# wkh923/m3pc

Measured on AMD Instinct MI355X. Metric: MPC plan-steps/sec (N=1024, H=16, hopper-medium-v2); independent plan steps, 3 in flight, higher is better.
Workload: dtype bf16; 1 GPU; hopper-medium-v2 shapes (S=11,A=3) rtg_guiding N=1024 H=16 T=32 bf16 candidate pass + fp32 policy pass + fp32 re-score (arg-max and multinomial draw certified under the calibrated bound delta, 8.4 candidates re-scored on average); 3 independent plan steps in flight (policy pass / candidate pass / re-score of neighbouring steps on different streams); window resident in HBM; candidates_per_gpu=1024, global_candidates=1024, horizon=16, traj_length=32, steps_in_flight=3, settle_steps=24, parallelism=1 GPU

## Files before the change

m3pc_amd/csrc/attn_bf16.hip:

```cpp
#include <cstdio>

#include "kernels.h"

namespace m3pc {

typedef float f32x16 __attribute__((ext_vector_type(16)));
typedef __bf16 bf16x8 __attribute__((ext_vector_type(8)));
typedef __bf16 bf16x4 __attribute__((ext_vector_type(4)));
typedef unsigned int u32x4 __attribute__((ext_vector_type(4)));
typedef short s16x4 __attribute__((ext_vector_type(4)));
typedef short s16x8 __attribute__((ext_vector_type(8)));
typedef float f32x4v __attribute__((ext_vector_type(4)));

template <int HDT, int NCH>
__global__ __launch_bounds__(256) void attn_bf16_kernel(AttnP p) {
    constexpr int HD = HDT * 32;
    constexpr int ROWB = HD * 2 + 16;
    constexpr int NS = HD / 16;
    constexpr int CPR = HD / 8;
    extern __shared__ __attribute__((aligned(16))) char lds[];

    const int tid = threadIdx.x, lane = tid & 63, wid = tid >> 6;
    const int nthr = blockDim.x, nw = nthr >> 6;
    const int b = blockIdx.x, head = blockIdx.y, qg = blockIdx.z;
// ... 190 lines not shown
    const int Lk = p.L1 + p.L2;
    const int l31 = lane & 31, lh = lane >> 5;
    const bf16_t* Qb = (const bf16_t*)p.Q + b * p.q_bstride + head * HD;
    const bf16_t* K1 = (const bf16_t*)p.K1 + b * p.kv1_bstride + head * HD;
    const bf16_t* V1 = (const bf16_t*)p.V1 + b * p.kv1_bstride + head * HD;
    const bf16_t* K2 = p.K2 ? (const bf16_t*)p.K2 + head * HD : nullptr;
    const bf16_t* V2 = p.V2 ? (const bf16_t*)p.V2 + head * HD : nullptr;
    const u32x4 zero4 = {0u, 0u, 0u, 0u};
    const int Lq1p = (p.Lq + 31) & ~31;
    const bf16_t* Q2b = p.Q2 ? (const bf16_t*)p.Q2 + head * HD : nullptr;

    const int qi = q0 + wid * 32 + l31;
    const bf16_t* qrow = nullptr;
    if (qi < p.Lq)
        qrow = Qb + (long long)qi * p.ldq;
    else if (Q2b && qi >= Lq1p && qi - Lq1p < p.Lq2)
        qrow = Q2b + (long long)(qi - Lq1p) * p.ldq2;
    u32x4 qf[NS];
#pragma unroll
    for (int s = 0; s < NS; ++s) {
        qf[s] = zero4;
        if (qrow) qf[s] = *(const u32x4*)(qrow + 16 * s + 8 * lh);
    }
    f32x16 sacc[NKT];
#pragma unroll
    for (int jt = 0; jt < NKT; ++jt)
#pragma unroll
        for (int e = 0; e < 16; ++e) sacc[jt][e] = 0.f;
#pragma unroll
    for (int pr = 0; pr < NKT / 2; ++pr) {
        u32x4 kf[2][NS];
#pragma unroll
        for (int t = 0; t < 2; ++t) {
            const int j = (2 * pr + t) * 32 + l31;
            const bf16_t* krow = j < p.L1 ? K1 + (long long)j * p.ldkv1 : (j < Lk ? K2 + (long long)(j - p.L1) * p.ldkv2 : nullptr);
#pragma unroll
            for (int s = 0; s < NS; ++s) {
                kf[t][s] = zero4;
                if (krow) kf[t][s] = *(const u32x4*)(krow + 16 * s + 8 * lh);
            }
        }
#pragma unroll
        for (int t = 0; t < 2; ++t)
            if ((2 * pr + t) * 32 < Lk) {
#pragma unroll
                for (int s = 0; s < NS; ++s)
                    sacc[2 * pr + t] = __builtin_amdgcn_mfma_f32_32x32x16_bf16(__builtin_bit_cast(bf16x8, kf[t][s]),
                                                                               __builtin_bit_cast(bf16x8, qf[s]), sacc[2 * pr + t], 0, 0, 0);
            }
    }
    u32x4 vv[VPT];
#pragma unroll
    for (int i = 0; i < VPT; ++i) {
        const int x = tid + i * NTHR, r = x / CPR, kc = x % CPR;
        vv[i] = zero4;
        if (r < p.L1)
            vv[i] = *(const u32x4*)(V1 + (long long)r * p.ldkv1 + kc * 8);
        else if (r < Lk)
            vv[i] = *(const u32x4*)(V2 + (long long)(r - p.L1) * p.ldkv2 + kc * 8);
    }

    float m = -INFINITY;
#pragma unroll
    for (int jt = 0; jt < NKT; ++jt)
#pragma unroll
        for (int e = 0; e < 16; ++e) {
            const int j = jt * 32 + (e & 3) + 8 * (e >> 2) + 4 * lh;
            const float v = (j < Lk) ? sacc[jt][e] * p.scale : -INFINITY;
            sacc[jt][e] = v;
            m = fmaxf(m, v);
        }
    m = fmaxf(m, __shfl_xor(m, 32));
    float l = 0.f;
#pragma unroll
    for (int jt = 0; jt < NKT; ++jt)
#pragma unroll
        for (int e = 0; e < 16; ++e) {
            const float v = __builtin_amdgcn_exp2f((sacc[jt][e] - m) * 1.44269504088896340736f);
            sacc[jt][e] = v;
            l += v;
        }
    l += __shfl_xor(l, 32);
    float inv = 1.0f / l;
    if (p.pre_m) {
        float mp = -INFINITY, lp = 0.f;
        if (qi < p.Lq) {
            mp = p.pre_m[head * p.Lq + qi];
            lp = p.pre_l[head * p.Lq + qi];
        }
        const float mt = fmaxf(m, mp);
        const float a = __builtin_amdgcn_exp2f((m - mt) * 1.44269504088896340736f);
        const float bs = __builtin_amdgcn_exp2f((mp - mt) * 1.44269504088896340736f);
        const float lt = l * a + lp * bs;
        inv = a / lt;
        if (lh == 0) fbuf[wid * 32 + l31] = bs / lt;
    }
#pragma unroll
    for (int i = 0; i < VPT; ++i) {
        const int x = tid + i * NTHR, r = x / CPR, kc = x % CPR;
        *(u32x4*)(lds + r * ROWB + kc * 16) = vv[i];
    }
    __syncthreads();

    f32x16 oacc[HDT];
#pragma unroll
    for (int d = 0; d < HDT; ++d)
#pragma unroll
        for (int e = 0; e < 16; ++e) oacc[d][e] = 0.f;
    const int gi = lane & 15;
    const int tr_off = (gi >> 2) * ROWB + (((lane >> 4) & 1) * 16 + (gi & 3) * 4) * 2;
#pragma unroll
    for (int jt = 0; jt < NKT; ++jt) {
        if (jt * 32 < Lk) {
#pragma unroll
            for (int s2 = 0; s2 < 2; ++s2) {
                bf16x8 pa;
#pragma unroll
                for (int e = 0; e < 8; ++e) pa[e] = (bf16_t)(sacc[jt][8 * s2 + e] * inv);
                const int kb = jt * 32 + 16 * s2 + 4 * lh;
#pragma unroll
                for (int d = 0; d < HDT; ++d) {
                    const char* base = lds + kb * ROWB + d * 64 + tr_off;
                    const s16x4 v0 = __builtin_amdgcn_ds_read_tr16_b64_v4i16((s16x4 __attribute__((address_space(3)))*)(base));
                    const s16x4 v1 =
                        __builtin_amdgcn_ds_read_tr16_b64_v4i16((s16x4 __attribute__((address_space(3)))*)(base + 8 * ROWB));
                    const s16x8 vb = __builtin_shufflevector(v0, v1, 0, 1, 2, 3, 4, 5, 6, 7);
                    oacc[d] = __builtin_amdgcn_mfma_f32_32x32x16_bf16(pa, __builtin_bit_cast(bf16x8, vb), oacc[d], 0, 0, 0);
                }
            }
        }
    }
    bf16_t* Ob = (bf16_t*)p.O + b * p.o_bstride + head * HD;
#pragma unroll
    for (int e = 0; e < 16; ++e) {
        const int i = q0 + wid * 32 + (e & 3) + 8 * (e >> 2) + 4 * lh;
        int orow = -1;
        if (i < p.Lq)
            orow = p.orow1 + i;
        else if (Q2b && i >= Lq1p && i - Lq1p < p.Lq2)
            orow = p.orow2 + i - Lq1p;
        if (orow >= 0) {
            if (p.pre_m) {
                const float f = fbuf[i - q0];
                const float* po = p.pre_O + ((long long)head * p.Lq + i) * HD;
#pragma unroll
                for (int d = 0; d < HDT; ++d) oacc[d][e] = fmaf(f, po[d * 32 + l31], oacc[d][e]);
            }
#pragma unroll
            for (int d = 0; d < HDT; ++d) Ob[(long long)orow * p.ldo + d * 32 + l31] = (bf16_t)oacc[d][e];
        }
    }
}
namespace {
constexpr int APIPE_NR = 52, APIPE_IMG = APIPE_NR * 256, APIPE_BUF = 3 * APIPE_IMG;
}
template <int N1, int SH>
__global__ __launch_bounds__(192, 2) void attn_bf16_pipe_kernel(AttnP p, int n_items) {
#if defined(__HIP_DEVICE_COMPILE__)
    constexpr int HD = 128, NS = 8, HDT = 4;
    constexpr int Lk = N1 + SH;
    constexpr int NP_OWN = (N1 + 3) / 4, NP_SH = SH ? (Lk + 3) / 4 - N1 / 4 : 0;
    constexpr int NDMA = NP_OWN + 2 * (NP_OWN + NP_SH);
    static_assert(NDMA <= 63 && Lk <= APIPE_NR && (SH == 0 || (SH == 32 && N1 <= APIPE_NR - 32)), "shapes");
    extern __shared__ __attribute__((aligned(16))) char lds[];
    typedef __attribute__((address_space(3))) void* lptr_t;
    const int tid = threadIdx.x, lane = tid & 63;
    const int wid = __builtin_amdgcn_readfirstlane(tid >> 6);
    const int l31 = lane & 31, lh = lane >> 5;
    constexpr int QROW0 = SH ? 32 : 0;

    {
        const u32x4 z = {0u, 0u, 0u, 0u};
        constexpr int NZ = (APIPE_NR - Lk) * 16;
        for (int i = tid; i < 2 * NZ; i += 192) *(u32x4*)(lds + (i / NZ) * APIPE_BUF + Lk * 256 + (i % NZ) * 16) = z;
    }
    const int r4 = lane >> 4, c16 = lane & 15;
    const int n_mine = ((int)blockIdx.x < n_items) ? (n_items - 1 - (int)blockIdx.x) / (int)gridDim.x + 1 : 0;
    const int stride = gridDim.x;
    asm volatile("s_waitcnt lgkmcnt(0)\n\ts_barrier" ::: "memory");

    if (wid == 2) {
        auto voff = [&](int ld, int odd) { return (unsigned)(r4 * ld * 2 + ((c16 ^ (4 * odd + r4)) << 4)); };
        const unsigned vq[2] = {voff(p.ldq, 0), voff(p.ldq, 1)};
        const unsigned vk[2] = {voff(p.ldkv1, 0), voff(p.ldkv1, 1)}, vk2[2] = {voff(p.ldkv2, 0), voff(p.ldkv2, 1)};
        auto seg_dma = [&](const bf16_t* src, int ld, const unsigned (&v)[2], char* img, auto r0_c, auto l_c, auto aux_c) {
            constexpr int R0 = decltype(r0_c)::value, L = decltype(l_c)::value, AUX = decltype(aux_c)::value;
            if (L == 0) return;
            const __amdgpu_buffer_rsrc_t rs = __builtin_amdgcn_make_buffer_rsrc((void*)(src - (long long)R0 * ld), 0, (unsigned)((R0 + L) * ld * 2), 0x00020000);
#pragma unroll
            for (int pc = R0 / 4; pc <= (R0 + L - 1) / 4; ++pc) {
                const bool lo = 4 * pc >= R0 ? true : 4 * pc + r4 >= R0;
                const bool hi = 4 * pc + 3 < R0 + L ? true : 4 * pc + r4 < R0 + L;
                if (lo && hi) __builtin_amdgcn_raw_ptr_buffer_load_lds(rs, (lptr_t)(img + pc * 1024), 16, v[pc & 1], pc * 4 * ld * 2, 0, AUX);
            }
        };
        using I0 = std::integral_constant<int, 0>;
        auto issue = [&](int it, int buf) {
            if (p.no_pipe == 3) return;
            const int b = it >> 2, head = it & 3;
            char* const B = lds + buf * APIPE_BUF;
            using AS = std::integral_constant<int, M3PC_STREAM_AUX>;
            seg_dma((const bf16_t*)p.K1 + b * p.kv1_bstride + head * HD, p.ldkv1, vk, B + APIPE_IMG, I0{}, std::integral_constant<int, N1>{}, AS{});
            seg_dma((const bf16_t*)p.K2 + head * HD, p.ldkv2, vk2, B + APIPE_IMG, std::integral_constant<int, N1>{}, std::integral_constant<int, SH>{}, I0{});
            seg_dma((const bf16_t*)p.Q + b * p.q_bstride + head * HD, p.ldq, vq, B + 2 * APIPE_IMG, std::integral_constant<int, QROW0>{}, std::integral_constant<int, N1>{}, AS{});
            seg_dma((const bf16_t*)p.V1 + b * p.kv1_bstride + head * HD, p.ldkv1, vk, B, I0{}, std::integral_constant<int, N1>{}, AS{});
            seg_dma((const bf16_t*)p.V2 + head * HD, p.ldkv2, vk2, B, std::integral_constant<int, N1>{}, std::integral_constant<int, SH>{}, I0{});
        };
        if (n_mine > 0) issue(blockIdx.x, 0);
        if (n_mine > 1) issue(blockIdx.x + stride, 1);
        for (int k = 0; k < n_mine; ++k) {
            if (k == 0 && n_mine > 1) asm volatile("s_waitcnt vmcnt(%0)" ::"n"(NDMA) : "memory");
            else asm volatile("s_waitcnt vmcnt(0)" ::: "memory");
            asm volatile("s_barrier" ::: "memory");
            if (k >= 1 && k + 1 < n_mine) issue(blockIdx.x + (k + 1) * stride, (k + 1) & 1);
            asm volatile("s_barrier" ::: "memory");
        }
        return;
    }
    const int qi = wid * 32 + l31;
    const int sw = l31 & 7;
    const int gi = lane & 15;
    long long st_[8] = {0, 0, 0, 0, 0, 0, 0, 0};
    u32x4 qf[NS];
    if (SH && wid == 1) {
        const bf16_t* qrow = (const bf16_t*)p.Q2 + (blockIdx.x % p.n_head) * HD + (long long)l31 * p.ldq2 + 8 * lh;
#pragma unroll
        for (int s = 0; s < NS; ++s) qf[s] = *(const u32x4*)(qrow + 16 * s);
    }
    for (int k = 0; k < n_mine; ++k) {
        const int it = blockIdx.x + k * stride;
        const char* const B = lds + (k & 1) * APIPE_BUF;
        asm volatile("s_barrier" ::: "memory");
        if (p.stamps && k == 2) st_[0] = __builtin_readcyclecounter();
        if (p.no_pipe == 2) {
            asm volatile("s_barrier" ::: "memory");
            continue;
        }
        const unsigned vbase = (unsigned)(uintptr_t)(const __attribute__((address_space(3))) char*)B;
        const char* const Ki = B + APIPE_IMG;
        const char* const Qi = B + 2 * APIPE_IMG;
        if (SH == 0 || wid == 0) {
#pragma unroll
            for (int s = 0; s < NS; ++s) qf[s] = *(const u32x4*)(Qi + (QROW0 + qi) * 256 + (((2 * s + lh) ^ sw) << 4));
        }
        f32x16 sacc[2];
#pragma unroll
        for (int t = 0; t < 2; ++t)
#pragma unroll
            for (int e = 0; e < 16; ++e) sacc[t][e] = 0.f;
#pragma unroll
        for (int s = 0; s < NS; ++s)
#pragma unroll
            for (int t = 0; t < 2; ++t) {
                const u32x4 kf = *(const u32x4*)(Ki + (32 * t + l31) * 256 + (((2 * s + lh) ^ sw) << 4));
                sacc[t] = __builtin_amdgcn_mfma_f32_32x32x16_bf16(__builtin_bit_cast(bf16x8, kf), __builtin_bit_cast(bf16x8, qf[s]), sacc[t], 0, 0, 0);
            }
        asm volatile("" : "+v"(sacc[0]), "+v"(sacc[1]));
        if (p.stamps && k == 2) st_[1] = __builtin_readcyclecounter();
        float m = -INFINITY;
#pragma unroll
        for (int jt = 0; jt < 2; ++jt)
#pragma unroll
            for (int e = 0; e < 16; ++e) {
                if (jt * 32 + (e & 3) + 8 * (e >> 2) >= Lk) continue;
                const int j = jt * 32 + (e & 3) + 8 * (e >> 2) + 4 * lh;
                const float v = (jt * 32 + (e & 3) + 8 * (e >> 2) + 4 < Lk || j < Lk) ? sacc[jt][e] * p.scale : -INFINITY;
                sacc[jt][e] = v;
                m = fmaxf(m, v);
            }
        m = fmaxf(m, __shfl_xor(m, 32));
        float l = 0.f;
#pragma unroll
        for (int jt = 0; jt < 2; ++jt)
#pragma unroll
            for (int e = 0; e < 16; ++e) {
                if (jt * 32 + (e & 3) + 8 * (e >> 2) >= Lk) {
                    sacc[jt][e] = 0.f;
                    continue;
                }
                const float v = __builtin_amdgcn_exp2f((sacc[jt][e] - m) * 1.44269504088896340736f);
                sacc[jt][e] = v;
                l += v;
            }
        l += __shfl_xor(l, 32);
        const float inv = 1.0f / l;
        asm volatile("" : "+v"(l));
        if (p.stamps && k == 2) st_[2] = __builtin_readcyclecounter();
        f32x16 oacc[HDT];
#pragma unroll
        for (int d = 0; d < HDT; ++d)
#pragma unroll
            for (int e = 0; e < 16; ++e) oacc[d][e] = 0.f;
        s16x4 tv[2][2 * HDT];
        auto tr_reads = [&](int n, s16x4 (&v)[2 * HDT]) {
            const int kr = 16 * n + 4 * lh + (gi >> 2);
#pragma unroll
            for (int d = 0; d < HDT; ++d) {
                const int bo = d * 64 + ((lane >> 4) & 1) * 32 + (gi & 3) * 8;
                const unsigned a0 = vbase + kr * 256 + ((((bo >> 4) ^ (kr & 7)) << 4) | (bo & 15));
                const unsigned a1 = vbase + (kr + 8) * 256 + ((((bo >> 4) ^ ((kr + 8) & 7)) << 4) | (bo & 15));
                asm volatile("ds_read_b64_tr_b16 %0, %1" : "=v"(v[2 * d]) : "v"(a0));
                asm volatile("ds_read_b64_tr_b16 %0, %1" : "=v"(v[2 * d + 1]) : "v"(a1));
            }
        };
        tr_reads(0, tv[0]);
#pragma unroll
        for (int n = 0; n < 4; ++n) {
            const int jt = n >> 1, s2 = n & 1;
            bf16x8 pa;
#pragma unroll
            for (int e = 0; e < 8; ++e) pa[e] = (bf16_t)(sacc[jt][8 * s2 + e] * inv);
            s16x4(&cur)[2 * HDT] = tv[n & 1];
            if (n < 3) {
                tr_reads(n + 1, tv[(n + 1) & 1]);
                asm volatile("s_waitcnt lgkmcnt(8)" : "+v"(cur[0]), "+v"(cur[1]), "+v"(cur[2]), "+v"(cur[3]), "+v"(cur[4]), "+v"(cur[5]), "+v"(cur[6]), "+v"(cur[7]));
            } else {
                asm volatile("s_waitcnt lgkmcnt(0)" : "+v"(cur[0]), "+v"(cur[1]), "+v"(cur[2]), "+v"(cur[3]), "+v"(cur[4]), "+v"(cur[5]), "+v"(cur[6]), "+v"(cur[7]));
            }
#pragma unroll
            for (int d = 0; d < HDT; ++d) {
                const s16x8 vb = __builtin_shufflevector(cur[2 * d], cur[2 * d + 1], 0, 1, 2, 3, 4, 5, 6, 7);
                oacc[d] = __builtin_amdgcn_mfma_f32_32x32x16_bf16(__builtin_bit_cast(bf16x8, vb), pa, oacc[d], 0, 0, 0);
            }
        }
        asm volatile("" : "+v"(oacc[0]), "+v"(oacc[1]), "+v"(oacc[2]), "+v"(oacc[3]));
        if (p.stamps && k == 2) st_[3] = __builtin_readcyclecounter();
        {
            char* const Oi = (char*)Qi;
            const int orow_i = SH == 0 ? qi : (wid == 0 ? 32 + qi : qi - 32);
            if (SH == 0 ? qi < APIPE_NR : (wid == 1 || qi < N1)) {
#pragma unroll
                for (int d = 0; d < HDT; ++d)
#pragma unroll
                    for (int q = 0; q < 4; ++q) {
                        bf16x4 w;
#pragma unroll
                        for (int i = 0; i < 4; ++i) w[i] = (bf16_t)oacc[d][4 * q + i];
                        *(bf16x4*)(Oi + orow_i * 256 + (((4 * d + q) ^ (orow_i & 7)) << 4) + 8 * lh) = w;
                    }
            }
        }
        if (p.stamps && k == 2) st_[4] = __builtin_readcyclecounter();
        constexpr int NPC_LO = 8, NPC_HI = APIPE_NR / 4 - 8;
        const bool low_rows = SH == 0 ? wid == 0 : wid == 1;
        u32x4 ov[NPC_LO];
#pragma unroll
        for (int j = 0; j < NPC_LO; ++j) {
            const int pc = low_rows ? j : (j < NPC_HI ? 8 + j : 8 + NPC_HI - 1);
            ov[j] = *(const u32x4*)(Qi + (4 * pc + r4) * 256 + c16 * 16);
        }
        asm volatile("s_waitcnt lgkmcnt(0)\n\ts_barrier" ::: "memory");
        if (p.stamps && k == 2) st_[5] = __builtin_readcyclecounter();
        {
            const int b = it >> 2, head = it & 3;
            const __amdgpu_buffer_rsrc_t o_rs = __builtin_amdgcn_make_buffer_rsrc(
                (void*)((bf16_t*)p.O + b * p.o_bstride + head * HD), 0, 0x7fffffffu, 0x00020000);
#pragma unroll
            for (int j = 0; j < NPC_LO; ++j) {
                const int pc = low_rows ? j : (j < NPC_HI ? 8 + j : 8 + NPC_HI - 1);
                const int row = 4 * pc + r4;
                const unsigned off = row < Lk ? (unsigned)((SH ? row : p.orow1 + row) * p.ldo * 2) : 0x80000000u;
                __builtin_amdgcn_raw_buffer_store_b128(ov[j], o_rs, off + ((c16 ^ (row & 7)) << 4), 0, M3PC_STREAM_AUX);
            }
        }
        if (p.stamps && k == 2) st_[6] = __builtin_readcyclecounter();
    }
    if (p.stamps && (int)blockIdx.x == 37 && lane == 0)
        for (int i = 0; i < 7; ++i) p.stamps[wid * 8 + i] = st_[i];
#endif
}
template <int N1>
__global__ __launch_bounds__(192, 1) void attn_bf16_pipe_dec_kernel(AttnP p, int n_items) {
#if defined(__HIP_DEVICE_COMPILE__)
    constexpr int HD = 128, NS = 8, HDT = 4;
    constexpr int Lk = N1;
    constexpr int NPC = (N1 + 3) / 4;
    constexpr int NDMA = 2 * 2 * NPC;
    constexpr int DBUF = 2 * APIPE_IMG;
    static_assert(NDMA <= 63 && Lk <= APIPE_NR, "shapes");
    extern __shared__ __attribute__((aligned(16))) char lds[];
    typedef __attribute__((address_space(3))) void* lptr_t;
    const int tid = threadIdx.x, lane = tid & 63;
    const int wid = __builtin_amdgcn_readfirstlane(tid >> 6);
    const int l31 = lane & 31, lh = lane >> 5;
    {
        const u32x4 z = {0u, 0u, 0u, 0u};
        constexpr int NZ = (APIPE_NR - Lk) * 16;
        for (int i = tid; i < 4 * NZ; i += 192) *(u32x4*)(lds + (i / NZ) * DBUF + Lk * 256 + (i % NZ) * 16) = z;
    }
    const int r4 = lane >> 4, c16 = lane & 15;
    const int stride = gridDim.x;
    const int n_mine = ((int)blockIdx.x < n_items) ? (n_items - 1 - (int)blockIdx.x) / stride + 1 : 0;
    const int n_rounds = (n_mine + 1) / 2;
    const int head = blockIdx.x & 3;
    asm volatile("s_waitcnt lgkmcnt(0)\n\ts_barrier" ::: "memory");

    if (wid == 2) {
        const unsigned v[2] = {(unsigned)(r4 * p.ldkv1 * 2 + ((c16 ^ r4) << 4)), (unsigned)(r4 * p.ldkv1 * 2 + ((c16 ^ (4 + r4)) << 4))};
        auto issue = [&](int r) {
            if (p.no_pipe == 3) return;
#pragma unroll
            for (int w = 0; w < 2; ++w) {
                int j = 2 * r + w;
                j = j < n_mine ? j : n_mine - 1;
                const int it = blockIdx.x + stride * j;
                char* const B = lds + (2 * w + (r & 1)) * DBUF;
                const bf16_t* kb = (const bf16_t*)p.K1 + (long long)(it >> 2) * p.kv1_bstride + head * HD;
                const bf16_t* vb = (const bf16_t*)p.V1 + (long long)(it >> 2) * p.kv1_bstride + head * HD;
                const __amdgpu_buffer_rsrc_t krs = __builtin_amdgcn_make_buffer_rsrc((void*)kb, 0, (unsigned)(N1 * p.ldkv1 * 2), 0x00020000);
                const __amdgpu_buffer_rsrc_t vrs = __builtin_amdgcn_make_buffer_rsrc((void*)vb, 0, (unsigned)(N1 * p.ldkv1 * 2), 0x00020000);
#pragma unroll
                for (int pc = 0; pc < NPC; ++pc) {
                    const bool ok = 4 * pc + 3 < N1 ? true : 4 * pc + r4 < N1;
                    if (ok) {
                        __builtin_amdgcn_raw_ptr_buffer_load_lds(krs, (lptr_t)(B + APIPE_IMG + pc * 1024), 16, v[pc & 1], pc * 4 * p.ldkv1 * 2, 0, M3PC_STREAM_AUX);
                        __builtin_amdgcn_raw_ptr_buffer_load_lds(vrs, (lptr_t)(B + pc * 1024), 16, v[pc & 1], pc * 4 * p.ldkv1 * 2, 0, M3PC_STREAM_AUX);
                    }
                }
            }
        };
        if (n_rounds > 0) issue(0);
        if (n_rounds > 1) issue(1);
        for (int r = 0; r < n_rounds; ++r) {
            if (r == 0 && n_rounds > 1) asm volatile("s_waitcnt vmcnt(%0)" ::"n"(NDMA) : "memory");
            else asm volatile("s_waitcnt vmcnt(0)" ::: "memory");
            asm volatile("s_barrier" ::: "memory");
            if (r >= 1 && r + 1 < n_rounds) issue(r + 1);
            asm volatile("s_barrier" ::: "memory");
        }
        return;
    }
    const int qi = l31;
    const int sw = l31 & 7;
    const int gi = lane & 15;
    u32x4 qf[NS];
    {
        const bf16_t* qrow = (const bf16_t*)p.Q + head * HD + (long long)(qi < p.Lq ? qi : 0) * p.ldq + 8 * lh;
#pragma unroll
        for (int s = 0; s < NS; ++s) qf[s] = *(const u32x4*)(qrow + 16 * s);
    }
    float mp = -INFINITY, lp = 0.f;
    f32x4v po[HDT][4];
    if (qi < p.Lq) {
        mp = p.pre_m[head * p.Lq + qi];
        lp = p.pre_l[head * p.Lq + qi];
    }
    {
        const float* prow = p.pre_O + ((long long)head * p.Lq + (qi < p.Lq ? qi : 0)) * HD + 4 * lh;
#pragma unroll
        for (int d = 0; d < HDT; ++d)
#pragma unroll
            for (int q = 0; q < 4; ++q) po[d][q] = *(const f32x4v*)(prow + d * 32 + 8 * q);
    }
    const unsigned ooff_base = qi < p.Lq ? 0u : 0x80000000u;
    (void)ooff_base;
    for (int r = 0; r < n_rounds; ++r) {
        const int j = 2 * r + wid;
        const bool have = j < n_mine;
        const int it = blockIdx.x + stride * (have ? j : 0);
        const char* const B = lds + (2 * wid + (r & 1)) * DBUF;
        asm volatile("s_barrier" ::: "memory");
        if (have && p.no_pipe != 2) {
            const unsigned vbase = (unsigned)(uintptr_t)(const __attribute__((address_space(3))) char*)B;
            const char* const Ki = B + APIPE_IMG;
            f32x16 sacc[2];
#pragma unroll
            for (int t = 0; t < 2; ++t)
#pragma unroll
                for (int e = 0; e < 16; ++e) sacc[t][e] = 0.f;
#pragma unroll
            for (int s = 0; s < NS; ++s)
#pragma unroll
                for (int t = 0; t < 2; ++t) {
                    const u32x4 kf = *(const u32x4*)(Ki + (32 * t + l31) * 256 + (((2 * s + lh) ^ sw) << 4));
                    sacc[t] = __builtin_amdgcn_mfma_f32_32x32x16_bf16(__builtin_bit_cast(bf16x8, kf), __builtin_bit_cast(bf16x8, qf[s]), sacc[t], 0, 0, 0);
                }
            float m = -INFINITY;
#pragma unroll
            for (int jt = 0; jt < 2; ++jt)
#pragma unroll
                for (int e = 0; e < 16; ++e) {
                    if (jt * 32 + (e & 3) + 8 * (e >> 2) >= Lk) continue;
                    const int jj = jt * 32 + (e & 3) + 8 * (e >> 2) + 4 * lh;
                    const float v = (jt * 32 + (e & 3) + 8 * (e >> 2) + 4 < Lk || jj < Lk) ? sacc[jt][e] * p.scale : -INFINITY;
                    sacc[jt][e] = v;
                    m = fmaxf(m, v);
                }
            m = fmaxf(m, __shfl_xor(m, 32));
            float l = 0.f;
#pragma unroll
            for (int jt = 0; jt < 2; ++jt)
#pragma unroll
                for (int e = 0; e < 16; ++e) {
                    if (jt * 32 + (e & 3) + 8 * (e >> 2) >= Lk) {
                        sacc[jt][e] = 0.f;
                        continue;
                    }
                    const float v = __builtin_amdgcn_exp2f((sacc[jt][e] - m) * 1.44269504088896340736f);
                    sacc[jt][e] = v;
                    l += v;
                }
            l += __shfl_xor(l, 32);
            const float mt = fmaxf(m, mp);
            const float a = __builtin_amdgcn_exp2f((m - mt) * 1.44269504088896340736f);
            const float bs = __builtin_amdgcn_exp2f((mp - mt) * 1.44269504088896340736f);
            const float lt = l * a + lp * bs;
            const float inv = a / lt;
            const float fpre = bs / lt;
            f32x16 oacc[HDT];
#pragma unroll
            for (int d = 0; d < HDT; ++d)
#pragma unroll
                for (int e = 0; e < 16; ++e) oacc[d][e] = 0.f;
            s16x4 tv[2][2 * HDT];
            auto tr_reads = [&](int n, s16x4 (&v)[2 * HDT]) {
                const int kr = 16 * n + 4 * lh + (gi >> 2);
#pragma unroll
                for (int d = 0; d < HDT; ++d) {
                    const int bo = d * 64 + ((lane >> 4) & 1) * 32 + (gi & 3) * 8;
                    const unsigned a0 = vbase + kr * 256 + ((((bo >> 4) ^ (kr & 7)) << 4) | (bo & 15));
                    const unsigned a1 = vbase + (kr + 8) * 256 + ((((bo >> 4) ^ ((kr + 8) & 7)) << 4) | (bo & 15));
// ... 411 lines not shown
            }
        float m = -INFINITY;
#pragma unroll
        for (int jt = 0; jt < NKT; ++jt)
#pragma unroll
            for (int e = 0; e < 16; ++e) {
                if (jt * 32 + (e & 3) + 8 * (e >> 2) >= Lk) continue;
                const int j = jt * 32 + (e & 3) + 8 * (e >> 2) + 4 * lh;
                const float v = (jt * 32 + (e & 3) + 8 * (e >> 2) + 4 < Lk || j < Lk) ? sacc[jt][e] * p.scale : -INFINITY;
                sacc[jt][e] = v;
                m = fmaxf(m, v);
            }
        m = fmaxf(m, __shfl_xor(m, 32));
        float l = 0.f;
#pragma unroll
        for (int jt = 0; jt < NKT; ++jt)
#pragma unroll
            for (int e = 0; e < 16; ++e) {
                if (jt * 32 + (e & 3) + 8 * (e >> 2) >= Lk) {
                    sacc[jt][e] = 0.f;
                    continue;
                }
                const float v = __builtin_amdgcn_exp2f((sacc[jt][e] - m) * 1.44269504088896340736f);
                sacc[jt][e] = v;
                l += v;
            }
        l += __shfl_xor(l, 32);
        float inv = 1.0f / l, fpre = 0.f;
        if constexpr (PRE) {
            const float mt = fmaxf(m, mp);
            const float a = __builtin_amdgcn_exp2f((m - mt) * 1.44269504088896340736f);
            const float bs = __builtin_amdgcn_exp2f((mp - mt) * 1.44269504088896340736f);
            const float lt = l * a + lp * bs;
            inv = a / lt;
            fpre = bs / lt;
        }
        u32x4 pa[NSTEP];
#pragma unroll
        for (int n = 0; n < NSTEP; ++n) {
            bf16x8 w;
#pragma unroll
            for (int e = 0; e < 8; ++e) w[e] = (bf16_t)(sacc[n >> 1][8 * (n & 1) + e] * inv);
            pa[n] = __builtin_bit_cast(u32x4, w);
            asm volatile("" : "+v"(pa[n]));
        }
        f32x16 oacc[HDT];
#pragma unroll
        for (int d = 0; d < HDT; ++d)
#pragma unroll
            for (int e = 0; e < 16; ++e) oacc[d][e] = 0.f;
        s16x4 tv[2][2 * HDT];
        unsigned tb[HDT];
        {
            const int kr = 4 * lh + (gi >> 2);
#pragma unroll
            for (int d = 0; d < HDT; ++d) {
                const int bo = d * 64 + ((lane >> 4) & 1) * 32 + (gi & 3) * 8;
                tb[d] = vbase + kr * 256 + ((((bo >> 4) ^ (kr & 7)) << 4) | (bo & 15));
            }
        }
        auto tr_reads = [](auto n_c, const unsigned (&tb)[HDT], s16x4 (&v)[2 * HDT]) {
            constexpr int n = decltype(n_c)::value;
#pragma unroll
            for (int d = 0; d < HDT; ++d) {
                asm volatile("ds_read_b64_tr_b16 %0, %1 offset:%2" : "=v"(v[2 * d]) : "v"(tb[d]), "n"(n * 4096));
                asm volatile("ds_read_b64_tr_b16 %0, %1 offset:%2" : "=v"(v[2 * d + 1]) : "v"(tb[d]), "n"(n * 4096 + 2048));
            }
        };
        tr_reads(std::integral_constant<int, 0>{}, tb, tv[0]);
        static_for<NSTEP>([&](auto n_c) {
            constexpr int n = decltype(n_c)::value;
            s16x4(&cur)[2 * HDT] = tv[n & 1];
            if constexpr (n < NSTEP - 1) {
                tr_reads(std::integral_constant<int, n + 1>{}, tb, tv[(n + 1) & 1]);
                asm volatile("s_waitcnt lgkmcnt(8)" : "+v"(cur[0]), "+v"(cur[1]), "+v"(cur[2]), "+v"(cur[3]), "+v"(cur[4]), "+v"(cur[5]), "+v"(cur[6]), "+v"(cur[7]));
            } else {
                asm volatile("s_waitcnt lgkmcnt(0)" : "+v"(cur[0]), "+v"(cur[1]), "+v"(cur[2]), "+v"(cur[3]), "+v"(cur[4]), "+v"(cur[5]), "+v"(cur[6]), "+v"(cur[7]));
            }
#pragma unroll
            for (int d = 0; d < HDT; ++d) {
                const s16x8 vb = __builtin_shufflevector(cur[2 * d], cur[2 * d + 1], 0, 1, 2, 3, 4, 5, 6, 7);
                oacc[d] = __builtin_amdgcn_mfma_f32_32x32x16_bf16(__builtin_bit_cast(bf16x8, vb), __builtin_bit_cast(bf16x8, pa[n]), oacc[d], 0, 0, 0);
            }
        });
        {
            char* const Oi = (char*)Qi;
            if (qrow_i < WPIPE_NR) {
#pragma unroll
                for (int d = 0; d < HDT; ++d)
#pragma unroll
                    for (int q = 0; q < 4; ++q) {
                        bf16x4 w;
#pragma unroll
                        for (int i = 0; i < 4; ++i) w[i] = (bf16_t)(PRE ? fmaf(fpre, po[PRE ? d : 0][q][i], oacc[d][4 * q + i]) : oacc[d][4 * q + i]);
                        *(bf16x4*)(Oi + qrow_i * 256 + (((4 * d + q) ^ sw) << 4) + 8 * lh) = w;
                    }
            }
        }
        u32x4 ov[8];
#pragma unroll
        for (int j = 0; j < 8; ++j) {
            const int pc = 8 * wid + j < WPIPE_NR / 4 ? 8 * wid + j : WPIPE_NR / 4 - 1;
            ov[j] = *(const u32x4*)(Qi + (4 * pc + r4) * 256 + c16 * 16);
        }
        asm volatile("s_waitcnt lgkmcnt(0)\n\ts_barrier" ::: "memory");
        {
            const __amdgpu_buffer_rsrc_t o_rs = __builtin_amdgcn_make_buffer_rsrc(
                (void*)((bf16_t*)p.O + (long long)(it >> 2) * p.o_bstride + head * HD), 0, 0x7fffffffu, 0x00020000);
#pragma unroll
            for (int j = 0; j < 8; ++j) {
                const int pc = 8 * wid + j;
                const int row = 4 * pc + r4;
                const unsigned off = pc < WPIPE_NR / 4 && row < n_out ? (unsigned)((SHQ && !PRE ? row : p.orow1 + row) * p.ldo * 2) : 0x80000000u;
                __builtin_amdgcn_raw_buffer_store_b128(ov[j], o_rs, off + ((c16 ^ (row & 7)) << 4), 0, 0);
            }
        }
    }
#endif
}
template <typename K>
static bool lds_opt_in(K kernel, int bytes) {
    static bool done[64] = {}, ok[64] = {};
    int dev = 0;
    if (hipGetDevice(&dev) != hipSuccess || dev < 0 || dev >= 64) return false;
    if (!done[dev]) {
        ok[dev] = hipFuncSetAttribute((const void*)kernel, hipFuncAttributeMaxDynamicSharedMemorySize, bytes) == hipSuccess;
        done[dev] = true;
    }
    return ok[dev];
}
template <int N1, int N2>
static bool launch_pipe_mix(const AttnP& p, hipStream_t st) {
    const int n_items = p.batch * p.n_head;
    const int grid = n_items < 256 ? n_items : 256;
    constexpr int LDSB = 2 * ((N2 + 3) / 4) * 1024 + 4 * (2 * APIPE_IMG + 1024);
    static_assert(LDSB <= 160 * 1024, "LDS");
    if (!lds_opt_in(attn_bf16_pipe_mix_kernel<N1, N2>, LDSB)) return false;
    M3PC_ATTN_PICK(23);
    hipLaunchKernelGGL((attn_bf16_pipe_mix_kernel<N1, N2>), dim3(grid), dim3(192), LDSB, st, p, n_items);
    return true;
}
template <int N1>
static bool launch_pipe_dec(const AttnP& p, hipStream_t st) {
    const int n_items = p.batch * p.n_head;
    const int grid = n_items < 256 ? n_items : 256;
    if (!lds_opt_in(attn_bf16_pipe_dec_kernel<N1>, 8 * APIPE_IMG)) return false;
    M3PC_ATTN_PICK(22);
    hipLaunchKernelGGL((attn_bf16_pipe_dec_kernel<N1>), dim3(grid), dim3(192), 8 * APIPE_IMG, st, p, n_items);
    return true;
}
template <int N1, int SH>
static bool launch_pipe(const AttnP& p, hipStream_t st) {
    const int n_items = p.batch * p.n_head;
    int cap = 512;
#ifdef M3PC_LAB
    static const int env_cap = M3PC_ENV("M3PC_ATTN_PIPE_GRID") ? atoi(M3PC_ENV("M3PC_ATTN_PIPE_GRID")) : 0;
    if (env_cap > 0) cap = env_cap;
#endif
    cap -= cap % p.n_head;
    const int grid = n_items < cap ? n_items : cap;
    if (!lds_opt_in(attn_bf16_pipe_kernel<N1, SH>, 2 * APIPE_BUF)) return false;
    size_t lds_bytes = 2 * APIPE_BUF;
#ifdef M3PC_LAB
    static const int env_lds = M3PC_ENV("M3PC_ATTN_PIPE_LDS") ? atoi(M3PC_ENV("M3PC_ATTN_PIPE_LDS")) : 0;
    if (env_lds > 0) lds_bytes = env_lds;
#endif
    M3PC_ATTN_PICK(SH == 0 ? 20 : 21);
    hipLaunchKernelGGL((attn_bf16_pipe_kernel<N1, SH>), dim3(grid), dim3(192), lds_bytes, st, p, n_items);
    return true;
}
static bool wide_off() {
    static const bool off = M3PC_ENV("M3PC_NO_ATTN_PIPE_WIDE") != nullptr;
    return off;
}
template <int NQ1, int SHQ, int NK1, int SHK, bool PRE>
static bool launch_pipe_wide(const AttnP& p, hipStream_t st) {
    const int n_items = p.batch * p.n_head;
    const int grid = n_items < 256 ? n_items : 256;
    if (!lds_opt_in(attn_bf16_pipe_wide_kernel<NQ1, SHQ, NK1, SHK, PRE>, WPIPE_LDS)) return false;
    constexpr int NTHR = ((NQ1 + SHQ + 31) / 32 + 1) * 64;
    M3PC_ATTN_PICK(PRE ? 26 : SHQ == 0 ? 24 : 25);
    hipLaunchKernelGGL((attn_bf16_pipe_wide_kernel<NQ1, SHQ, NK1, SHK, PRE>), dim3(grid), dim3(NTHR), WPIPE_LDS, st, p, n_items);
    return true;
}
static bool try_pipe(const AttnP& p, hipStream_t st) {
    if (p.hd != 128 || p.n_head != 4 || p.no_pipe == 1 || p.batch * p.n_head < 1024) return false;
    if (p.pre_m) {
        if (p.q_bstride != 0 || p.Q2 || p.K2 || p.Lq < 1 || p.L2 != 0 || !p.pre_l || !p.pre_O) return false;
        if (((uintptr_t)p.Q | (uintptr_t)p.K1 | (uintptr_t)p.V1 | (uintptr_t)p.O | (uintptr_t)p.pre_O) & 15) return false;
        if ((p.ldq | p.ldkv1 | p.ldo) % 8 || (p.kv1_bstride | p.o_bstride) % 8) return false;
        if ((long long)128 * p.ldkv1 * 2 >= 0x7fffffffLL || (long long)128 * p.ldo * 2 >= 0x7fffffffLL) return false;
        if (p.Lq <= 32 && p.L1 == 49) return launch_pipe_dec<49>(p, st);
        if (p.Lq > 32 && p.Lq <= 64 && p.L1 == 97 && !wide_off()) return launch_pipe_wide<0, 64, 97, 0, true>(p, st);
        return false;
    }
    if (((uintptr_t)p.Q | (uintptr_t)p.K1 | (uintptr_t)p.V1 | (uintptr_t)p.O) & 15) return false;
    if ((p.ldq | p.ldkv1 | p.ldo) % 8 || (p.q_bstride | p.kv1_bstride | p.o_bstride) % 8) return false;
    if (p.Q2 && p.K2 && p.V2 && p.Lq >= 1 && p.Lq <= 4 && p.Lq + p.Lq2 <= 32 && p.L1 == 49 && p.L2 == 79 && p.orow1 == 0 && p.orow2 == p.Lq &&
        !(((uintptr_t)p.Q2 | (uintptr_t)p.K2 | (uintptr_t)p.V2) & 15) && (p.ldq2 | p.ldkv2) % 8 == 0 && (long long)128 * p.ldkv2 * 2 < 0x7fffffffLL &&
        (long long)64 * p.ldkv1 * 2 < 0x7fffffffLL && (long long)64 * p.ldo * 2 < 0x7fffffffLL)
        return launch_pipe_mix<49, 79>(p, st);
    if ((long long)64 * p.ldq * 2 >= 0x7fffffffLL || (long long)64 * p.ldkv1 * 2 >= 0x7fffffffLL || (long long)64 * p.ldo * 2 >= 0x7fffffffLL) return false;
    if (!p.Q2 && !p.K2 && p.Lq == 49 && p.L1 == 49 && p.L2 == 0 && p.orow1 >= 0) {
        return launch_pipe<49, 0>(p, st);
    }
    if ((long long)128 * p.ldq * 2 >= 0x7fffffffLL || (long long)128 * p.ldkv1 * 2 >= 0x7fffffffLL || (long long)128 * p.ldo * 2 >= 0x7fffffffLL) return false;
    if (!p.Q2 && !p.K2 && p.Lq == 97 && p.L1 == 97 && p.L2 == 0 && p.orow1 >= 0 && !wide_off()) return launch_pipe_wide<97, 0, 97, 0, false>(p, st);
    if (p.Q2 && p.K2 && p.V2 && p.Lq == 33 && p.L1 == 33 && p.Lq2 == 64 && p.L2 == 64 && p.orow1 == 64 && p.orow2 == 0 && !wide_off() &&
        !(((uintptr_t)p.Q2 | (uintptr_t)p.K2 | (uintptr_t)p.V2) & 15) && (p.ldq2 | p.ldkv2) % 8 == 0 && (long long)128 * p.ldkv2 * 2 < 0x7fffffffLL) {
        return launch_pipe_wide<33, 64, 33, 64, false>(p, st);
    }
    if (p.Q2 && p.K2 && p.V2 && p.Lq == 17 && p.L1 == 17 && p.Lq2 == 32 && p.L2 == 32 && p.orow1 == 32 && p.orow2 == 0 &&
        !(((uintptr_t)p.Q2 | (uintptr_t)p.K2 | (uintptr_t)p.V2) & 15) && (p.ldq2 | p.ldkv2) % 8 == 0 && (long long)64 * p.ldkv2 * 2 < 0x7fffffffLL) {
        return launch_pipe<17, 32>(p, st);
    }
    return false;
}

template <int HDT>
__global__ __launch_bounds__(64, 4) void attn_bf16_pack2_kernel(AttnP p) {
    constexpr int HD = HDT * 32;
    constexpr int ROWB = HD * 2 + 16;
    constexpr int NS = HD / 16;
    constexpr int CPR = HD / 8;
    __shared__ __attribute__((aligned(16))) char lds[32 * ROWB];
    const int lane = threadIdx.x, l31 = lane & 31, lh = lane >> 5;
    const int head = blockIdx.y, b0 = 2 * blockIdx.x;
    const u32x4 zero4 = {0u, 0u, 0u, 0u};
    const int wb = b0 + (l31 >> 4), tk = l31 & 15;
    const bool wok = wb < p.batch;
    const bf16_t* qrow = wok && tk < p.Lq ? (const bf16_t*)p.Q + (long long)wb * p.q_bstride + head * HD + (long long)tk * p.ldq : nullptr;
    const bf16_t* krow = wok && tk < p.L1 ? (const bf16_t*)p.K1 + (long long)wb * p.kv1_bstride + head * HD + (long long)tk * p.ldkv1 : nullptr;
    u32x4 qf[NS], kf[NS];
#pragma unroll
    for (int s = 0; s < NS; ++s) {
        qf[s] = zero4;
        if (qrow) qf[s] = *(const u32x4*)(qrow + 16 * s + 8 * lh);
    }
#pragma unroll
    for (int s = 0; s < NS; ++s) {
        kf[s] = zero4;
        if (krow) kf[s] = *(const u32x4*)(krow + 16 * s + 8 * lh);
    }
    f32x16 sacc;
#pragma unroll
    for (int e = 0; e < 16; ++e) sacc[e] = 0.f;
#pragma unroll
    for (int s = 0; s < NS; ++s)
        sacc = __builtin_amdgcn_mfma_f32_32x32x16_bf16(__builtin_bit_cast(bf16x8, kf[s]), __builtin_bit_cast(bf16x8, qf[s]), sacc, 0, 0, 0);
    constexpr int VPT = 32 * CPR / 64;
    u32x4 vv[VPT];
#pragma unroll
    for (int i = 0; i < VPT; ++i) {
        const int x = lane + i * 64, r = x / CPR, kc = x % CPR;
        const int vb = b0 + (r >> 4), vt = r & 15;
        vv[i] = zero4;
        if (vb < p.batch && vt < p.L1) vv[i] = *(const u32x4*)((const bf16_t*)p.V1 + (long long)vb * p.kv1_bstride + head * HD + (long long)vt * p.ldkv1 + kc * 8);
    }
    float m = -INFINITY;
#pragma unroll
    for (int e = 0; e < 16; ++e) {
        const int j = (e & 3) + 8 * (e >> 2) + 4 * lh;
        const float v = ((j >> 4) == (l31 >> 4) && (j & 15) < p.L1) ? sacc[e] * p.scale : -INFINITY;
        sacc[e] = v;
        m = fmaxf(m, v);
    }
    m = fmaxf(m, __shfl_xor(m, 32));
    float l = 0.f;
#pragma unroll
    for (int e = 0; e < 16; ++e) {
        const float v = __builtin_amdgcn_exp2f((sacc[e] - m) * 1.44269504088896340736f);
        sacc[e] = v;
        l += v;
    }
    l += __shfl_xor(l, 32);
    const float inv = 1.0f / l;
#pragma unroll
    for (int i = 0; i < VPT; ++i) {
        const int x = lane + i * 64, r = x / CPR, kc = x % CPR;
        *(u32x4*)(lds + r * ROWB + kc * 16) = vv[i];
    }
    __syncthreads();
    f32x16 oacc[HDT];
#pragma unroll
    for (int d = 0; d < HDT; ++d)
#pragma unroll
        for (int e = 0; e < 16; ++e) oacc[d][e] = 0.f;
    const int gi = lane & 15;
    const int tr_off = (gi >> 2) * ROWB + (((lane >> 4) & 1) * 16 + (gi & 3) * 4) * 2;
#pragma unroll
    for (int s2 = 0; s2 < 2; ++s2) {
        bf16x8 pa;
#pragma unroll
        for (int e = 0; e < 8; ++e) pa[e] = (bf16_t)(sacc[8 * s2 + e] * inv);
        const int kb = 16 * s2 + 4 * lh;
#pragma unroll
        for (int d = 0; d < HDT; ++d) {
            const char* base = lds + kb * ROWB + d * 64 + tr_off;
            const s16x4 v0 = __builtin_amdgcn_ds_read_tr16_b64_v4i16((s16x4 __attribute__((address_space(3)))*)(base));
            const s16x4 v1 = __builtin_amdgcn_ds_read_tr16_b64_v4i16((s16x4 __attribute__((address_space(3)))*)(base + 8 * ROWB));
            const s16x8 vb = __builtin_shufflevector(v0, v1, 0, 1, 2, 3, 4, 5, 6, 7);
            oacc[d] = __builtin_amdgcn_mfma_f32_32x32x16_bf16(pa, __builtin_bit_cast(bf16x8, vb), oacc[d], 0, 0, 0);
        }
    }
#pragma unroll
    for (int e = 0; e < 16; ++e) {
        const int i = (e & 3) + 8 * (e >> 2) + 4 * lh;
        const int ob = b0 + (i >> 4), ot = i & 15;
        if (ob < p.batch && ot < p.Lq) {
            bf16_t* Ob = (bf16_t*)p.O + (long long)ob * p.o_bstride + head * HD + (long long)(p.orow1 + ot) * p.ldo;
#pragma unroll
            for (int d = 0; d < HDT; ++d) Ob[d * 32 + l31] = (bf16_t)oacc[d][e];
        }
    }
}

template <int HDT, int NW, int NKT>
static void launch_direct(const AttnP& p, int slots, hipStream_t st) {
    const size_t smem = (size_t)NKT * 32 * (HDT * 64 + 16) + NW * 32 * sizeof(float);
    const int qgroups = (slots + NW * 32 - 1) / (NW * 32);
    M3PC_ATTN_PICK(30 + 3 * (HDT == 1 ? 0 : HDT == 2 ? 1 : 2) + (NW == 1 ? 0 : NKT == 2 ? 1 : 2));
// ... 95 lines not shown
```

Measured before the change: 882.8 plan-steps/s.

## Drop Q from LDS pipeline, prefetch Q to registers, fit three blocks per CU

The pipelined attention kernel no longer DMAs Q into shared memory. Each compute wave now loads its Q fragment straight from global into registers, prefetching the next item's Q during the current one. Freeing the Q image cuts LDS per block from three images to two per buffer, so launch bounds go to three workgroups per CU and the grid cap rises to 768. It also restructures the PV loop into per-d transposed reads with finer lgkmcnt waits, reuses the K image for the O staging with an extra barrier, and uses ds_bpermute for the cross-half reductions. In exchange it adds register pressure, extra barriers per item, and direct global Q loads.

```diff
diff --git a/m3pc_amd/csrc/attn_bf16.hip b/m3pc_amd/csrc/attn_bf16.hip
--- a/m3pc_amd/csrc/attn_bf16.hip
+++ b/m3pc_amd/csrc/attn_bf16.hip
@@ -366,40 +366,49 @@
     }
 }
 namespace {
-constexpr int APIPE_NR = 52, APIPE_IMG = APIPE_NR * 256, APIPE_BUF = 3 * APIPE_IMG;
+constexpr int APIPE_NR = 52, APIPE_IMG = APIPE_NR * 256;
+constexpr int APIPE_KV = 2 * APIPE_IMG;
+constexpr int APIPE_LDS = 2 * APIPE_KV;
+static_assert(APIPE_NR % 4 == 0 && 3 * APIPE_LDS <= 160 * 1024, "three workgroups of attn_bf16_pipe_kernel per CU");
+}
+static __device__ __forceinline__ int lane_now() {
+    int lane;
+    asm volatile("v_mbcnt_lo_u32_b32 %0, -1, 0\n\tv_mbcnt_hi_u32_b32 %0, -1, %0" : "=v"(lane));
+    return lane;
 }
 template <int N1, int SH>
-__global__ __launch_bounds__(192, 2) void attn_bf16_pipe_kernel(AttnP p, int n_items) {
+__global__ __launch_bounds__(192, 3) void attn_bf16_pipe_kernel(AttnP p, int n_items) {
 #if defined(__HIP_DEVICE_COMPILE__)
     constexpr int HD = 128, NS = 8, HDT = 4;
     constexpr int Lk = N1 + SH;
     constexpr int NP_OWN = (N1 + 3) / 4, NP_SH = SH ? (Lk + 3) / 4 - N1 / 4 : 0;
-    constexpr int NDMA = NP_OWN + 2 * (NP_OWN + NP_SH);
+    constexpr int NDMA = 2 * (NP_OWN + NP_SH);
     static_assert(NDMA <= 63 && Lk <= APIPE_NR && (SH == 0 || (SH == 32 && N1 <= APIPE_NR - 32)), "shapes");
+    static_assert(((Lk + 3) / 4) * 1024 <= APIPE_IMG && 64 * 256 <= APIPE_KV && N1 >= 64 - APIPE_NR && N1 >= 1 && N1 <= 32 + 32 * (SH == 0), "LDS addressing");
     extern __shared__ __attribute__((aligned(16))) char lds[];
     typedef __attribute__((address_space(3))) void* lptr_t;
     const int tid = threadIdx.x, lane = tid & 63;
     const int wid = __builtin_amdgcn_readfirstlane(tid >> 6);
     const int l31 = lane & 31, lh = lane >> 5;
-    constexpr int QROW0 = SH ? 32 : 0;
 
     {
         const u32x4 z = {0u, 0u, 0u, 0u};
         constexpr int NZ = (APIPE_NR - Lk) * 16;
-        for (int i = tid; i < 2 * NZ; i += 192) *(u32x4*)(lds + (i / NZ) * APIPE_BUF + Lk * 256 + (i % NZ) * 16) = z;
-    }
-    const int r4 = lane >> 4, c16 = lane & 15;
+        for (int i = tid; i < 2 * NZ; i += 192) *(u32x4*)(lds + (i / NZ) * APIPE_KV + Lk * 256 + (i % NZ) * 16) = z;
+    }
     const int n_mine = ((int)blockIdx.x < n_items) ? (n_items - 1 - (int)blockIdx.x) / (int)gridDim.x + 1 : 0;
     const int stride = gridDim.x;
     asm volatile("s_waitcnt lgkmcnt(0)\n\ts_barrier" ::: "memory");
 
     if (wid == 2) {
+        const int ll = lane_now();
+        const int r4 = ll >> 4, c16 = ll & 15;
         auto voff = [&](int ld, int odd) { return (unsigned)(r4 * ld * 2 + ((c16 ^ (4 * odd + r4)) << 4)); };
-        const unsigned vq[2] = {voff(p.ldq, 0), voff(p.ldq, 1)};
         const unsigned vk[2] = {voff(p.ldkv1, 0), voff(p.ldkv1, 1)}, vk2[2] = {voff(p.ldkv2, 0), voff(p.ldkv2, 1)};
         auto seg_dma = [&](const bf16_t* src, int ld, const unsigned (&v)[2], char* img, auto r0_c, auto l_c, auto aux_c) {
             constexpr int R0 = decltype(r0_c)::value, L = decltype(l_c)::value, AUX = decltype(aux_c)::value;
             if (L == 0) return;
+            static_assert(R0 >= 0 && R0 + L <= APIPE_NR, "a piece past its image");
             const __amdgpu_buffer_rsrc_t rs = __builtin_amdgcn_make_buffer_rsrc((void*)(src - (long long)R0 * ld), 0, (unsigned)((R0 + L) * ld * 2), 0x00020000);
 #pragma unroll
             for (int pc = R0 / 4; pc <= (R0 + L - 1) / 4; ++pc) {
@@ -412,11 +421,10 @@
         auto issue = [&](int it, int buf) {
             if (p.no_pipe == 3) return;
             const int b = it >> 2, head = it & 3;
-            char* const B = lds + buf * APIPE_BUF;
+            char* const B = lds + buf * APIPE_KV;
             using AS = std::integral_constant<int, M3PC_STREAM_AUX>;
             seg_dma((const bf16_t*)p.K1 + b * p.kv1_bstride + head * HD, p.ldkv1, vk, B + APIPE_IMG, I0{}, std::integral_constant<int, N1>{}, AS{});
             seg_dma((const bf16_t*)p.K2 + head * HD, p.ldkv2, vk2, B + APIPE_IMG, std::integral_constant<int, N1>{}, std::integral_constant<int, SH>{}, I0{});
-            seg_dma((const bf16_t*)p.Q + b * p.q_bstride + head * HD, p.ldq, vq, B + 2 * APIPE_IMG, std::integral_constant<int, QROW0>{}, std::integral_constant<int, N1>{}, AS{});
             seg_dma((const bf16_t*)p.V1 + b * p.kv1_bstride + head * HD, p.ldkv1, vk, B, I0{}, std::integral_constant<int, N1>{}, AS{});
             seg_dma((const bf16_t*)p.V2 + head * HD, p.ldkv2, vk2, B, std::integral_constant<int, N1>{}, std::integral_constant<int, SH>{}, I0{});
         };
@@ -428,35 +436,51 @@
             asm volatile("s_barrier" ::: "memory");
             if (k >= 1 && k + 1 < n_mine) issue(blockIdx.x + (k + 1) * stride, (k + 1) & 1);
             asm volatile("s_barrier" ::: "memory");
+            asm volatile("s_barrier" ::: "memory");
         }
         return;
     }
-    const int qi = wid * 32 + l31;
-    const int sw = l31 & 7;
-    const int gi = lane & 15;
     long long st_[8] = {0, 0, 0, 0, 0, 0, 0, 0};
-    u32x4 qf[NS];
-    if (SH && wid == 1) {
+    int wid_s = wid;
+    asm volatile("" : "+s"(wid_s));
+    const bool q_own = SH == 0 || wid == 0;
+    auto q_load = [&](int it, int l31, int lh, u32x4(&q)[NS]) {
+        const char* qbase = (const char*)((const bf16_t*)p.Q + (long long)(it >> 2) * p.q_bstride + (it & 3) * HD);
+        const int qi = wid * 32 + l31;
+        const unsigned qoff = (unsigned)(((qi < N1 ? qi : N1 - 1) * p.ldq + 8 * lh) * 2);
+#pragma unroll
+        for (int s = 0; s < NS; ++s) q[s] = *(const u32x4*)(qbase + qoff + 32 * s);
+    };
+    u32x4 qn[NS] = {};
+    if (!q_own) {
         const bf16_t* qrow = (const bf16_t*)p.Q2 + (blockIdx.x % p.n_head) * HD + (long long)l31 * p.ldq2 + 8 * lh;
 #pragma unroll
-        for (int s = 0; s < NS; ++s) qf[s] = *(const u32x4*)(qrow + 16 * s);
-    }
+        for (int s = 0; s < NS; ++s) qn[s] = *(const u32x4*)(qrow + 16 * s);
+    } else if (n_mine > 0) {
+        q_load(blockIdx.x, l31, lh, qn);
+    }
+#pragma unroll
+    for (int s = 0; s < NS; ++s) asm volatile("" : "+v"(qn[s]));
     for (int k = 0; k < n_mine; ++k) {
+        const int lane = lane_now();
+        auto xor32 = [&](float x) { return __builtin_bit_cast(float, __builtin_amdgcn_ds_bpermute((lane ^ 32) << 2, __builtin_bit_cast(int, x))); };
+        const int l31 = lane & 31, lh = lane >> 5, r4 = lane >> 4, c16 = lane & 15, gi = lane & 15, sw = l31 & 7, qi = wid * 32 + l31;
+        const int krow1 = (32 + l31 < APIPE_NR ? 32 + l31 : APIPE_NR - 1) * 256;
         const int it = blockIdx.x + k * stride;
-        const char* const B = lds + (k & 1) * APIPE_BUF;
+        const char* const B = lds + (k & 1) * APIPE_KV;
         asm volatile("s_barrier" ::: "memory");
         if (p.stamps && k == 2) st_[0] = __builtin_readcyclecounter();
         if (p.no_pipe == 2) {
             asm volatile("s_barrier" ::: "memory");
+            asm volatile("s_barrier" ::: "memory");
             continue;
         }
         const unsigned vbase = (unsigned)(uintptr_t)(const __attribute__((address_space(3))) char*)B;
         const char* const Ki = B + APIPE_IMG;
-        const char* const Qi = B + 2 * APIPE_IMG;
-        if (SH == 0 || wid == 0) {
-#pragma unroll
-            for (int s = 0; s < NS; ++s) qf[s] = *(const u32x4*)(Qi + (QROW0 + qi) * 256 + (((2 * s + lh) ^ sw) << 4));
-        }
+        u32x4 qf[NS];
+#pragma unroll
+        for (int s = 0; s < NS; ++s) qf[s] = qn[s];
+        if (q_own && k + 1 < n_mine) q_load(it + stride, l31, lh, qn);
         f32x16 sacc[2];
 #pragma unroll
         for (int t = 0; t < 2; ++t)
@@ -466,7 +490,7 @@
         for (int s = 0; s < NS; ++s)
 #pragma unroll
             for (int t = 0; t < 2; ++t) {
-                const u32x4 kf = *(const u32x4*)(Ki + (32 * t + l31) * 256 + (((2 * s + lh) ^ sw) << 4));
+                const u32x4 kf = *(const u32x4*)(Ki + (t == 0 ? l31 * 256 : krow1) + (((2 * s + lh) ^ sw) << 4));
                 sacc[t] = __builtin_amdgcn_mfma_f32_32x32x16_bf16(__builtin_bit_cast(bf16x8, kf), __builtin_bit_cast(bf16x8, qf[s]), sacc[t], 0, 0, 0);
             }
         asm volatile("" : "+v"(sacc[0]), "+v"(sacc[1]));
@@ -482,7 +506,7 @@
                 sacc[jt][e] = v;
                 m = fmaxf(m, v);
             }
-        m = fmaxf(m, __shfl_xor(m, 32));
+        m = fmaxf(m, xor32(m));
         float l = 0.f;
 #pragma unroll
         for (int jt = 0; jt < 2; ++jt)
@@ -496,7 +520,7 @@
                 sacc[jt][e] = v;
                 l += v;
             }
-        l += __shfl_xor(l, 32);
+        l += xor32(l);
         const float inv = 1.0f / l;
         asm volatile("" : "+v"(l));
         if (p.stamps && k == 2) st_[2] = __builtin_readcyclecounter();
@@ -505,43 +529,41 @@
         for (int d = 0; d < HDT; ++d)
 #pragma unroll
             for (int e = 0; e < 16; ++e) oacc[d][e] = 0.f;
-        s16x4 tv[2][2 * HDT];
-        auto tr_reads = [&](int n, s16x4 (&v)[2 * HDT]) {
+        s16x4 tv[2 * HDT];
+        auto tr_reads = [&](int n, int d) {
             const int kr = 16 * n + 4 * lh + (gi >> 2);
+            const int bo = d * 64 + ((lane >> 4) & 1) * 32 + (gi & 3) * 8;
+            const unsigned a0 = vbase + kr * 256 + ((((bo >> 4) ^ (kr & 7)) << 4) | (bo & 15));
+            const unsigned a1 = vbase + (kr + 8) * 256 + ((((bo >> 4) ^ ((kr + 8) & 7)) << 4) | (bo & 15));
+            asm volatile("ds_read_b64_tr_b16 %0, %1" : "=v"(tv[2 * d]) : "v"(a0));
+            asm volatile("ds_read_b64_tr_b16 %0, %1" : "=v"(tv[2 * d + 1]) : "v"(a1));
+        };
+#pragma unroll
+        for (int d = 0; d < HDT; ++d) tr_reads(0, d);
+        bf16x8 pa[4];
+#pragma unroll
+        for (int n = 0; n < 4; ++n)
+#pragma unroll
+            for (int e = 0; e < 8; ++e) pa[n][e] = (bf16_t)(sacc[n >> 1][8 * (n & 1) + e] * inv);
+        asm volatile("" : "+v"(pa[0]), "+v"(pa[1]), "+v"(pa[2]), "+v"(pa[3]));
+#pragma unroll
+        for (int n = 0; n < 4; ++n) {
 #pragma unroll
             for (int d = 0; d < HDT; ++d) {
-                const int bo = d * 64 + ((lane >> 4) & 1) * 32 + (gi & 3) * 8;
-                const unsigned a0 = vbase + kr * 256 + ((((bo >> 4) ^ (kr & 7)) << 4) | (bo & 15));
-                const unsigned a1 = vbase + (kr + 8) * 256 + ((((bo >> 4) ^ ((kr + 8) & 7)) << 4) | (bo & 15));
-                asm volatile("ds_read_b64_tr_b16 %0, %1" : "=v"(v[2 * d]) : "v"(a0));
-                asm volatile("ds_read_b64_tr_b16 %0, %1" : "=v"(v[2 * d + 1]) : "v"(a1));
-            }
-        };
-        tr_reads(0, tv[0]);
-#pragma unroll
-        for (int n = 0; n < 4; ++n) {
-            const int jt = n >> 1, s2 = n & 1;
-            bf16x8 pa;
-#pragma unroll
-            for (int e = 0; e < 8; ++e) pa[e] = (bf16_t)(sacc[jt][8 * s2 + e] * inv);
-            s16x4(&cur)[2 * HDT] = tv[n & 1];
-            if (n < 3) {
-                tr_reads(n + 1, tv[(n + 1) & 1]);
-                asm volatile("s_waitcnt lgkmcnt(8)" : "+v"(cur[0]), "+v"(cur[1]), "+v"(cur[2]), "+v"(cur[3]), "+v"(cur[4]), "+v"(cur[5]), "+v"(cur[6]), "+v"(cur[7]));
-            } else {
-                asm volatile("s_waitcnt lgkmcnt(0)" : "+v"(cur[0]), "+v"(cur[1]), "+v"(cur[2]), "+v"(cur[3]), "+v"(cur[4]), "+v"(cur[5]), "+v"(cur[6]), "+v"(cur[7]));
-            }
-#pragma unroll
-            for (int d = 0; d < HDT; ++d) {
-                const s16x8 vb = __builtin_shufflevector(cur[2 * d], cur[2 * d + 1], 0, 1, 2, 3, 4, 5, 6, 7);
-                oacc[d] = __builtin_amdgcn_mfma_f32_32x32x16_bf16(__builtin_bit_cast(bf16x8, vb), pa, oacc[d], 0, 0, 0);
+                if (n < 3) asm volatile("s_waitcnt lgkmcnt(6)" : "+v"(tv[2 * d]), "+v"(tv[2 * d + 1]));
+                else asm volatile("s_waitcnt lgkmcnt(%2)" : "+v"(tv[2 * d]), "+v"(tv[2 * d + 1]) : "n"(2 * (HDT - 1 - d)));
+                const s16x8 vb = __builtin_shufflevector(tv[2 * d], tv[2 * d + 1], 0, 1, 2, 3, 4, 5, 6, 7);
+                oacc[d] = __builtin_amdgcn_mfma_f32_32x32x16_bf16(__builtin_bit_cast(bf16x8, vb), pa[n], oacc[d], 0, 0, 0);
+                if (n < 3) tr_reads(n + 1, d);
             }
         }
         asm volatile("" : "+v"(oacc[0]), "+v"(oacc[1]), "+v"(oacc[2]), "+v"(oacc[3]));
         if (p.stamps && k == 2) st_[3] = __builtin_readcyclecounter();
+        asm volatile("s_waitcnt lgkmcnt(0)\n\ts_barrier" ::: "memory");
         {
-            char* const Oi = (char*)Qi;
+            char* const Oi = (char*)Ki;
             const int orow_i = SH == 0 ? qi : (wid == 0 ? 32 + qi : qi - 32);
+            static_assert(SH == 0 || 32 + N1 <= APIPE_NR, "O rows inside the K image");
             if (SH == 0 ? qi < APIPE_NR : (wid == 1 || qi < N1)) {
 #pragma unroll
                 for (int d = 0; d < HDT; ++d)
@@ -561,7 +583,7 @@
 #pragma unroll
         for (int j = 0; j < NPC_LO; ++j) {
             const int pc = low_rows ? j : (j < NPC_HI ? 8 + j : 8 + NPC_HI - 1);
-            ov[j] = *(const u32x4*)(Qi + (4 * pc + r4) * 256 + c16 * 16);
+            ov[j] = *(const u32x4*)(Ki + (4 * pc + r4) * 256 + c16 * 16);
         }
         asm volatile("s_waitcnt lgkmcnt(0)\n\ts_barrier" ::: "memory");
         if (p.stamps && k == 2) st_[5] = __builtin_readcyclecounter();
@@ -579,8 +601,8 @@
         }
         if (p.stamps && k == 2) st_[6] = __builtin_readcyclecounter();
     }
-    if (p.stamps && (int)blockIdx.x == 37 && lane == 0)
-        for (int i = 0; i < 7; ++i) p.stamps[wid * 8 + i] = st_[i];
+    if (p.stamps && (int)blockIdx.x == 37 && lane_now() == 0)
+        for (int i = 0; i < 7; ++i) p.stamps[wid_s * 8 + i] = st_[i];
 #endif
 }
 template <int N1>
@@ -1298,21 +1320,16 @@
 template <int N1, int SH>
 static bool launch_pipe(const AttnP& p, hipStream_t st) {
     const int n_items = p.batch * p.n_head;
-    int cap = 512;
+    int cap = 768;
 #ifdef M3PC_LAB
     static const int env_cap = M3PC_ENV("M3PC_ATTN_PIPE_GRID") ? atoi(M3PC_ENV("M3PC_ATTN_PIPE_GRID")) : 0;
     if (env_cap > 0) cap = env_cap;
 #endif
     cap -= cap % p.n_head;
     const int grid = n_items < cap ? n_items : cap;
-    if (!lds_opt_in(attn_bf16_pipe_kernel<N1, SH>, 2 * APIPE_BUF)) return false;
-    size_t lds_bytes = 2 * APIPE_BUF;
-#ifdef M3PC_LAB
-    static const int env_lds = M3PC_ENV("M3PC_ATTN_PIPE_LDS") ? atoi(M3PC_ENV("M3PC_ATTN_PIPE_LDS")) : 0;
-    if (env_lds > 0) lds_bytes = env_lds;
-#endif
+    if (!lds_opt_in(attn_bf16_pipe_kernel<N1, SH>, APIPE_LDS)) return false;
     M3PC_ATTN_PICK(SH == 0 ? 20 : 21);
-    hipLaunchKernelGGL((attn_bf16_pipe_kernel<N1, SH>), dim3(grid), dim3(192), lds_bytes, st, p, n_items);
+    hipLaunchKernelGGL((attn_bf16_pipe_kernel<N1, SH>), dim3(grid), dim3(192), APIPE_LDS, st, p, n_items);
     return true;
 }
 static bool wide_off() {
```

Result: no change. 885.9 plan-steps/s, median of 3 (+0.3%).
